# finmath/finmath-lib-cuda-extensions

Hardware: AMD Instinct MI355X
Metric: Monte-Carlo path-ops/sec (fused RandomVariable stream) (higher is better)
Workload: dtype f32

## Files before the change

### finmath-lib-cuda-extensions_amd/host/hip_backend.hpp

```cpp
#pragma once
#include <cstdlib>
#include <cstring>
#include <memory>
#include "lmm.hpp"

namespace fmhost {

class BrownianMotionFromMersenneRandomNumbersHip final : public BrownianMotion {
public:
    BrownianMotionFromMersenneRandomNumbersHip(TimeDiscretization td, int numberOfFactors, int64_t numberOfPaths, int seed, int64_t pathOffset = 0)
        : td_(std::move(td)), factors_(numberOfFactors), paths_(numberOfPaths), offset_(pathOffset), seed_(seed) {}
    RV getBrownianIncrement(int timeIndex, int factor) const override {
        std::call_once(generated_, [this] { generate(); });
        return inc_.at((size_t)timeIndex * factors_ + factor);
    }
    const TimeDiscretization& getTimeDiscretization() const override { return td_; }
    int getNumberOfFactors() const override { return factors_; }
    int64_t getNumberOfPaths() const override { return paths_; }
    int getSeed() const { return seed_; }
    RV getRandomVariableForConstant(double value) const override { return RandomVariableHip::of(-std::numeric_limits<double>::infinity(), value); }
private:
    void generate() const {
        const int steps = td_.getNumberOfTimeSteps();
        std::vector<double> dt((size_t)steps);
        for (int i = 0; i < steps; ++i) dt[(size_t)i] = td_.getTimeStep(i);
        std::vector<fmhip_vec> h((size_t)steps * factors_);
        check(fmhip_bm_generate_mersenne_device(seed_, steps, factors_, paths_, offset_, dt.data(), h.data()));
        inc_.reserve(h.size());
        for (int i = 0; i < steps; ++i)
            for (int f = 0; f < factors_; ++f)
                inc_.push_back(RandomVariableHip::of(td_.getTime(i + 1), DeviceVector(h[(size_t)i * factors_ + f]), paths_));
    }
    TimeDiscretization td_;
    int factors_;
    int64_t paths_, offset_;
    int seed_;
    mutable std::vector<RV> inc_;
    mutable std::once_flag generated_;
};

inline lmm::Backend makeHipBackend(const RandomVariableFactory* factory, const BrownianMotion* brownianMotion, int chunk = 0, int stepsPerLaunch = 0, int jacobianBatch = 0) {
    lmm::Backend be;
    be.factory = factory;
    be.brownianMotion = brownianMotion;
    if (!(std::getenv("FMHIP_LMM_FLUSH") && std::getenv("FMHIP_LMM_FLUSH")[0] == '0'))
        be.flush = [] { check(fmhip_flush()); };
    if (!(std::getenv("FMHIP_LMM_HOLD") && std::getenv("FMHIP_LMM_HOLD")[0] == '0'))
        be.hold = [](bool h) { check(fmhip_fusion_hold(h ? 1 : 0, nullptr)); };
    if (chunk > 0) be.chunk = chunk;
    if (stepsPerLaunch > 0) be.stepsPerLaunch = stepsPerLaunch;
    be.jacobianBatch = jacobianBatch > 0 ? jacobianBatch : 8;
    if (!(std::getenv("FMHIP_LMM_CLONE") && std::getenv("FMHIP_LMM_CLONE")[0] == '0')) {
        auto handleOf = [](const RV& x) {
            auto p = dynamic_cast<const RandomVariableHip*>(x.get());
            if (!p || p->isDeterministic()) throw std::runtime_error("graph replication over a value that is not a device vector");
            return p->deviceVector().handle();
        };
        be.clone = [handleOf](const std::vector<RV>& roots, const std::vector<RV>& leafFrom, const std::vector<std::vector<RV>>& leafTo,
                              const std::vector<std::vector<double>>* scalars) {
            const int nRoots = (int)roots.size(), nMap = (int)leafFrom.size(), nCopies = (int)leafTo.size();
            std::vector<fmhip_vec> r, lf, lt, out((size_t)nRoots * nCopies);
            for (const RV& x : roots) r.push_back(handleOf(x));
            for (const RV& x : leafFrom) lf.push_back(handleOf(x));
            for (const auto& row : leafTo) { if ((int)row.size() != nMap) throw std::runtime_error("graph replication: ragged operand map"); for (const RV& x : row) lt.push_back(handleOf(x)); }
            std::vector<double> sc;
            int nScalars = 0;
            if (scalars) { nScalars = (int)(*scalars)[0].size(); for (const auto& row : *scalars) { if ((int)row.size() != nScalars) throw std::runtime_error("graph replication: ragged scalar lists"); sc.insert(sc.end(), row.begin(), row.end()); } }
            check(fmhip_graph_clone(r.data(), nRoots, nCopies, lf.data(), lt.data(), nMap, scalars ? sc.data() : nullptr, nScalars, out.data()));
            std::vector<std::vector<RV>> copies((size_t)nCopies);
            for (int c = 0; c < nCopies; ++c)
                for (int k = 0; k < nRoots; ++k)
                    copies[(size_t)c].push_back(RandomVariableHip::of(roots[(size_t)k]->getFiltrationTime(), DeviceVector(out[(size_t)c * nRoots + k]), roots[(size_t)k]->size()));
            return copies;
        };
        be.recordedScalars = [handleOf](const std::vector<RV>& roots) {
            std::vector<fmhip_vec> r;
            for (const RV& x : roots) r.push_back(handleOf(x));
            int n = 0;
            check(fmhip_graph_scalars(r.data(), (int)r.size(), nullptr, 0, &n));
            std::vector<double> sc((size_t)n);
            check(fmhip_graph_scalars(r.data(), (int)r.size(), sc.data(), n, &n));
            return sc;
        };
    }
    if (!(std::getenv("FMHIP_LMM_DISCARD") && std::getenv("FMHIP_LMM_DISCARD")[0] == '0'))
        be.valuesNotNeeded = [](const std::vector<RV>& v) {
            std::vector<fmhip_vec> h;
            for (const RV& x : v) { auto p = dynamic_cast<const RandomVariableHip*>(x.get()); if (p && !p->isDeterministic()) h.push_back(p->deviceVector().handle()); }
            if (!h.empty()) check(fmhip_vec_give_up_values(h.data(), (int)h.size()));
        };
    be.launches = [] { fmhip_engine_stats_t s; check(fmhip_engine_stats(&s)); return (long long)s.kernel_launches; };
    be.averages = [](const std::vector<RV>& v) { return getAverages(v); };
    if (!(std::getenv("FMHIP_LMM_ASYNC") && std::getenv("FMHIP_LMM_ASYNC")[0] == '0'))
        be.expectationsRunPending = true;
    if (!(std::getenv("FMHIP_LMM_ASYNC") && std::getenv("FMHIP_LMM_ASYNC")[0] == '0'))
        be.averagesAsync = [](const std::vector<RV>& v) -> std::function<std::vector<double>()> {
            std::vector<fmhip_vec> h;
            int64_t n = 0;
            for (const RV& x : v) {
                auto p = dynamic_cast<const RandomVariableHip*>(x.get());
                if (!p || p->isDeterministic()) { const std::vector<double> now = getAverages(v); return [now] { return now; }; }
                h.push_back(p->deviceVector().handle()); n = p->size();
            }
            const int count = (int)h.size();
            fmhip_ticket ticket = 0;
            check(fmhip_reduce_moments_batch_begin(h.data(), count, nullptr, &ticket));
            struct Owner { fmhip_ticket t = 0; int count = 0; bool ended = false;
                           Owner() = default; Owner(const Owner&) = delete; Owner& operator=(const Owner&) = delete;
                           ~Owner() { if (!ended && t) { std::vector<fmhip_moments> drop((size_t)count); (void)fmhip_reduce_moments_batch_end(t, drop.data(), count); } } };
            auto owner = std::make_shared<Owner>();
            owner->t = ticket; owner->count = count;
            return [owner, count, n] {
                std::vector<fmhip_moments> m((size_t)count);
                owner->ended = true;
                check(fmhip_reduce_moments_batch_end(owner->t, m.data(), count));
                std::vector<double> out((size_t)count);
                for (int k = 0; k < count; ++k) out[(size_t)k] = m[(size_t)k].sum / (double)n;
                return out;
            };
        };
    return be;
}

}
```

### finmath-lib-cuda-extensions_amd/host/lmm.hpp

```cpp
#pragma once
#include <algorithm>
#include <chrono>
#include <cmath>
#include <cstdio>
#include <atomic>
#include <thread>
#include <cstdlib>
#include <functional>
#include <string>
#include <vector>

#include "random_variable.hpp"

namespace fmhost { namespace lmm {


inline const std::vector<double>& atmNormalVolatilities() {
    static const std::vector<double> v = {
        0.00151, 0.00169, 0.0021, 0.00248, 0.00291, 0.00329, 0.00365, 0.004, 0.00437, 0.00466, 0.00527, 0.00571,
        0.00604, 0.00625, 0.0016, 0.00174, 0.00217, 0.00264, 0.00314, 0.00355, 0.00398, 0.00433, 0.00469,
        0.00493, 0.00569, 0.00607, 0.00627, 0.00645, 0.00182, 0.00204, 0.00238, 0.00286, 0.00339, 0.00384,
        0.00424, 0.00456, 0.00488, 0.0052, 0.0059, 0.00623, 0.0064, 0.00654, 0.00205, 0.00235, 0.00272, 0.0032,
        0.00368, 0.00406, 0.00447, 0.00484, 0.00515, 0.00544, 0.00602, 0.00629, 0.0064, 0.00646, 0.00279,
        0.00319, 0.0036, 0.00396, 0.00436, 0.00469, 0.00503, 0.0053, 0.00557, 0.00582, 0.00616, 0.00628,
// ... 23 lines not shown
        const double w = (time - t[k - 1]) / (t[k] - t[k - 1]);
        return std::exp(logdf[k - 1] + w * (logdf[k] - logdf[k - 1]));
    }
    double forward(double fixing, double period) const { return (df(fixing) / df(fixing + period) - 1.0) / period; }
    static DiscountCurve bootstrap() {
        const double maturities[] = { 0.5, 1, 2, 3, 4, 5, 6, 7, 8, 9, 10, 11, 12, 15, 20, 25, 30, 35, 40, 45, 50 };
        const double rates[] = { -0.00216, -0.00208, -0.00222, -0.00216, -0.0019, -0.0014, -0.00072, 0.00011, 0.00103, 0.00196, 0.00285,
                                 0.00367, 0.0044, 0.00604, 0.00733, 0.00767, 0.00773, 0.00765, 0.00752, 0.007138, 0.007 };
        DiscountCurve c;
        for (int i = 0; i < 21; ++i) {
            const double M = maturities[i], r = rates[i];
            c.t.push_back(M); c.logdf.push_back(c.logdf.back());
            auto swapValue = [&](double ld) {
                c.logdf.back() = ld;
                double annuity = 0.0;
                if (M < 1.0) annuity = M * c.df(M);
                else for (double tp = 1.0; tp <= M + 1e-9; tp += 1.0) annuity += c.df(tp);
                return 1.0 - c.df(M) - r * annuity;
            };
            double lo = -3.0, hi = 1.0;
            for (int it = 0; it < 200; ++it) { const double mid = 0.5 * (lo + hi); if (swapValue(mid) > 0) lo = mid; else hi = mid; }
            c.logdf.back() = 0.5 * (lo + hi);
        }
        return c;
    }
};

struct Swaption {
    double exercise = 0; int numberOfPeriods = 0; double swapPeriodLength = 0.5;
    std::vector<double> swapTenor; double swaprate = 0, targetVolatility = 0, annuity = 0;
};

struct Market {
    DiscountCurve curve = DiscountCurve::bootstrap();
    double lastTime = 40.0, dt = 0.5;
    TimeDiscretization timeDiscretization{ 0.0, 80, 0.5 };
    std::vector<Swaption> swaptions;
    Market() {
        const auto& vols = atmNormalVolatilities();
        for (size_t e = 0; e < atmExpiryYears().size(); ++e)
            for (size_t k = 0; k < atmTenorYears().size(); ++k) {
                const double exercise = std::round(atmExpiryYears()[e] / 0.25) * 0.25, tenor = atmTenorYears()[k];
                if (exercise < 1.0) continue;
                if (exercise + tenor > lastTime + 1e-9) continue;
                Swaption s;
                s.exercise = exercise; s.numberOfPeriods = (int)std::lround(tenor / 0.5);
                for (int p = 0; p <= s.numberOfPeriods; ++p) s.swapTenor.push_back(exercise + p * 0.5);
                double floating = 0.0, annuity = 0.0;
                for (int p = 0; p < s.numberOfPeriods; ++p) {
                    const double d = curve.df(s.swapTenor[p + 1]);
                    floating += curve.forward(s.swapTenor[p], 0.5) * 0.5 * d; annuity += 0.5 * d;
                }
                s.swaprate = floating / annuity; s.annuity = annuity;
                s.targetVolatility = vols[e * atmTenorYears().size() + k];
                swaptions.push_back(std::move(s));
            }
    }
    int numberOfLibors() const { return timeDiscretization.getNumberOfTimeSteps(); }
};

struct VolatilityModel {
    std::vector<double> grid{ 0.0, 1.0, 2.0, 5.0, 10.0, 20.0, 30.0, 40.0 };
    std::vector<double> parameter = std::vector<double>(64, 0.50 / 100);
    int bin(double x) const { int k = 0; while (k < 7 && grid[(size_t)k] < x - 1e-12) ++k; return k; }
    int parameterIndex(double time, double maturity) const { return bin(time) * 8 + bin(maturity - time); }
    double volatility(double time, double maturity) const { return maturity <= time + 1e-12 ? 0.0 : parameter[(size_t)parameterIndex(time, maturity)]; }
    std::vector<int> activeParameters(const Market& m) const {
        std::vector<char> used(64, 0);
        const auto& td = m.timeDiscretization;
        for (int i = 0; i < td.getNumberOfTimeSteps(); ++i)
            for (int j = i + 1; j < m.numberOfLibors(); ++j) used[(size_t)parameterIndex(td.getTime(i), td.getTime(j))] = 1;
        std::vector<int> idx;
        for (int k = 0; k < 64; ++k) if (used[(size_t)k]) idx.push_back(k);
        return idx;
    }
};


struct Simulation {
    std::vector<std::vector<RV>> libor;
    std::vector<RV> numeraire;
};

struct Backend {
    const RandomVariableFactory* factory = nullptr;
    const BrownianMotion* brownianMotion = nullptr;
    std::function<void()> flush = [] {};
    std::function<void(bool)> hold = [](bool) {};
    std::function<long long()> launches = [] { return 0LL; };
    std::function<std::vector<double>(const std::vector<RV>&)> averages = [](const std::vector<RV>& v) {
        std::vector<double> a; for (const RV& x : v) a.push_back(x->getAverage()); return a; };
    std::function<std::function<std::vector<double>()>(const std::vector<RV>&)> averagesAsync;
    bool expectationsRunPending = false;
    std::function<void(const std::vector<RV>&)> valuesNotNeeded;
    int chunk = 7;
    int stepsPerLaunch = 4;
    std::function<std::vector<std::vector<RV>>(const std::vector<RV>& roots, const std::vector<RV>& leafFrom, const std::vector<std::vector<RV>>& leafTo,
                                               const std::vector<std::vector<double>>* scalars)> clone;
    std::function<std::vector<double>(const std::vector<RV>& roots)> recordedScalars;
    int jacobianBatch = 1;
    bool keepAllStates = false;
    int threads = 1;
};

inline std::vector<Simulation> simulateMany(const Market& m, const std::vector<const VolatilityModel*>& vols, const Backend& be, int lastTimeIndex,
                                            const std::vector<char>* keep = nullptr) {
    const auto& td = m.timeDiscretization;
    const int n = m.numberOfLibors();
    const double delta = m.dt;
    const size_t K = vols.size();
    std::vector<Simulation> sims(K);
    for (Simulation& sim : sims) {
        sim.libor.resize((size_t)lastTimeIndex + 1);
        sim.numeraire.resize((size_t)lastTimeIndex + 1);
        sim.libor[0].resize((size_t)n);
        for (int j = 0; j < n; ++j) sim.libor[0][(size_t)j] = be.factory->createRandomVariable(0.0, m.curve.forward(td.getTime(j), delta));
        sim.numeraire[0] = be.factory->createRandomVariable(0.0, 1.0);
    }
    std::vector<RV> factorSum(K);
    const int S = std::max(1, be.stepsPerLaunch);
    static int cloneChecks = 0;
    for (int i0 = 0; i0 < lastTimeIndex;) {
        int i1 = std::min(i0 + S, lastTimeIndex);
        static const bool endAtKept = std::getenv("FMHIP_LMM_GROUPS_END_AT_KEPT") && std::getenv("FMHIP_LMM_GROUPS_END_AT_KEPT")[0] == '1';
        if (keep && endAtKept) for (int s2 = i0 + 1; s2 < i1; ++s2) if ((*keep)[(size_t)s2]) { i1 = s2; break; }
        const bool cloning = K > 1 && S > 1 && keep && be.clone && i0 >= 2;
        const size_t Krec = cloning ? 1 : K;
        if (S > 1) be.hold(true);
        for (int i = i0; i < i1; ++i) {
            const double t = td.getTime(i), dt = td.getTimeStep(i);
            const RV dW = be.brownianMotion->getBrownianIncrement(i, 0);
            for (size_t k = 0; k < Krec; ++k) {
                auto& cur = sims[k].libor[(size_t)i];
                auto& nxt = sims[k].libor[(size_t)i + 1];
                nxt.resize((size_t)n);
                for (int j = 0; j <= i && j < n; ++j) nxt[(size_t)j] = cur[(size_t)j];
                factorSum[k] = nullptr;
            }
            for (int j0 = i + 1; j0 < n; j0 += be.chunk) {
                const int j1 = std::min(n, j0 + be.chunk);
                for (size_t k = 0; k < Krec; ++k) {
                    auto& cur = sims[k].libor[(size_t)i];
                    auto& nxt = sims[k].libor[(size_t)i + 1];
                    for (int j = j0; j < j1; ++j) {
                        const double lambda = vols[k]->volatility(t, td.getTime(j));
                        const RV& L = cur[(size_t)j];
                        const RV transform = be.factory->createRandomVariable(lambda * delta)->discount(L, delta);
                        factorSum[k] = factorSum[k] ? factorSum[k]->add(transform) : transform;
                        const RV drift = factorSum[k]->mult(lambda);
                        nxt[(size_t)j] = L->addProduct(drift, dt)->addProduct(dW, lambda);
                    }
                }
                if (S == 1 && j1 - j0 == be.chunk) be.flush();
            }
            for (size_t k = 0; k < Krec; ++k)
                sims[k].numeraire[(size_t)i + 1] = sims[k].numeraire[(size_t)i]->accrue(sims[k].libor[(size_t)i][(size_t)i], delta);
            for (size_t k = 0; k < Krec; ++k) factorSum[k] = nullptr;
        }
        if (cloning) {
            std::vector<RV> roots, leafFrom;
            for (int j = i0 + 1; j < n; ++j) roots.push_back(sims[0].libor[(size_t)i1][(size_t)j]);
            for (int i = i0; i < i1; ++i) roots.push_back(sims[0].numeraire[(size_t)i + 1]);
            for (int s2 = i0 + 1; s2 < i1; ++s2)
                if (!keep || (*keep)[(size_t)s2]) for (int j = s2; j < n; ++j) roots.push_back(sims[0].libor[(size_t)s2][(size_t)j]);
            for (int j = i0; j < n; ++j) leafFrom.push_back(sims[0].libor[(size_t)i0][(size_t)j]);
            leafFrom.push_back(sims[0].numeraire[(size_t)i0]);
            auto scalarsOf = [&](const VolatilityModel& vol) {
                std::vector<double> sc;
                for (int i = i0; i < i1; ++i) {
                    const double t = td.getTime(i), dt = td.getTimeStep(i);
                    for (int j = i + 1; j < n; ++j) {
                        const double lambda = vol.volatility(t, td.getTime(j));
                        sc.push_back(delta); sc.push_back(1.0); sc.push_back(lambda * delta); sc.push_back(lambda); sc.push_back(dt); sc.push_back(lambda);
                    }
                    sc.push_back(delta);
                }
                return sc;
            };
            if (cloneChecks < 64 && be.recordedScalars) {
                ++cloneChecks;
                if (be.recordedScalars(roots) != scalarsOf(*vols[0])) throw std::runtime_error("lmm: the scalar list of the replicated Euler steps does not match the recording");
            }
            std::vector<std::vector<RV>> leafTo(K - 1);
            std::vector<std::vector<double>> scalars(K - 1);
            for (size_t k = 1; k < K; ++k) {
                for (int j = i0; j < n; ++j) leafTo[k - 1].push_back(sims[k].libor[(size_t)i0][(size_t)j]);
                leafTo[k - 1].push_back(sims[k].numeraire[(size_t)i0]);
                scalars[k - 1] = scalarsOf(*vols[k]);
            }
            const std::vector<std::vector<RV>> copies = be.clone(roots, leafFrom, leafTo, &scalars);
            for (size_t k = 1; k < K; ++k) {
                auto& nxt = sims[k].libor[(size_t)i1];
                nxt.resize((size_t)n);
                for (int j = 0; j <= i0 && j < n; ++j) nxt[(size_t)j] = sims[k].libor[(size_t)i0][(size_t)j];
                size_t r = 0;
                for (int j = i0 + 1; j < n; ++j) nxt[(size_t)j] = copies[k - 1][r++];
                for (int i = i0; i < i1; ++i) sims[k].numeraire[(size_t)i + 1] = copies[k - 1][r++];
                for (int s2 = i0 + 1; s2 < i1; ++s2)
                    if (!keep || (*keep)[(size_t)s2]) { auto& mid = sims[k].libor[(size_t)s2]; mid.resize((size_t)n); for (int j = s2; j < n; ++j) mid[(size_t)j] = copies[k - 1][r++]; }
            }
        }
        if (keep)
            for (int i = i0; i < i1; ++i)
                if (!(*keep)[(size_t)i])
                    for (size_t k = 0; k < K; ++k) { sims[k].libor[(size_t)i].clear(); sims[k].libor[(size_t)i].shrink_to_fit(); }
        if (S > 1) be.hold(false);
        be.flush();
        i0 = i1;
    }
    return sims;
}

inline Simulation simulate(const Market& m, const VolatilityModel& vol, const Backend& be, int lastTimeIndex) {
    return std::move(simulateMany(m, { &vol }, be, lastTimeIndex)[0]);
}

inline RV swaptionValue(const Market& m, const Simulation& sim, const Swaption& s) {
    const auto& td = m.timeDiscretization;
    const int exerciseIndex = td.getTimeIndex(s.exercise);
    RV value;
    for (int p = s.numberOfPeriods - 1; p >= 0; --p) {
        const int j = td.getTimeIndex(s.swapTenor[(size_t)p]);
        const RV& libor = sim.libor[(size_t)exerciseIndex][(size_t)j];
        const RV payoff = libor->sub(s.swaprate)->mult(s.swapPeriodLength);
        value = (value ? value->add(payoff) : payoff)->discount(libor, s.swapPeriodLength);
    }
    return value->floor(0.0)->div(sim.numeraire[(size_t)exerciseIndex]);
}
inline double bachelierAtmImpliedVolatility(double optionValue, double optionMaturity, double annuity) {
    return optionValue * std::sqrt(2.0 * 3.14159265358979323846) / (annuity * std::sqrt(optionMaturity));
}

struct Valuation { std::vector<double> modelVolatility; double seconds_simulation = 0, seconds_valuation = 0; long long launches_simulation = 0, launches_valuation = 0; };

struct PendingValuations {
    std::vector<std::function<std::vector<double>()>> expectations;
    std::vector<Valuation> out;
};

inline std::vector<Valuation> evaluateManyFinish(const Market& m, PendingValuations& p) {
    for (size_t k = 0; k < p.out.size(); ++k) {
        const std::vector<double> optionValues = p.expectations[k]();
        for (size_t q = 0; q < m.swaptions.size(); ++q)
            p.out[k].modelVolatility.push_back(bachelierAtmImpliedVolatility(optionValues[q], m.swaptions[q].exercise, m.swaptions[q].annuity));
    }
    return std::move(p.out);
}

inline PendingValuations evaluateManyBegin(const Market& m, const std::vector<const VolatilityModel*>& vols, const Backend& be) {
    using clk = std::chrono::steady_clock;
    const size_t K = vols.size();
    PendingValuations pending;
    std::vector<Valuation>& out = pending.out;
    out.resize(K);
    int lastIndex = 0;
    for (const Swaption& s : m.swaptions) lastIndex = std::max(lastIndex, m.timeDiscretization.getTimeIndex(s.exercise));
    const auto t0 = clk::now();
    const long long l0 = be.launches();
    std::vector<char> keep((size_t)lastIndex + 1, 0);
    for (const Swaption& s : m.swaptions) keep[(size_t)m.timeDiscretization.getTimeIndex(s.exercise)] = 1;
    const std::vector<Simulation> sims = simulateMany(m, vols, be, lastIndex, be.keepAllStates ? nullptr : &keep);
    const auto t1 = clk::now();
    const long long l1 = be.launches();
    std::vector<std::vector<RV>> values(K);
    if (K > 1 && be.clone) {
        be.hold(true);
        values[0].reserve(m.swaptions.size());
        for (const Swaption& s : m.swaptions) values[0].push_back(swaptionValue(m, sims[0], s));
        std::vector<RV> leafFrom;
        std::vector<std::vector<RV>> leafTo(K - 1);
        for (int e = 0; e <= lastIndex; ++e) {
            if (!keep[(size_t)e]) continue;
            for (size_t k = 0; k < K; ++k) {
                std::vector<RV>& dst = k == 0 ? leafFrom : leafTo[k - 1];
                for (int j = e; j < m.numberOfLibors(); ++j) dst.push_back(sims[k].libor[(size_t)e][(size_t)j]);
                dst.push_back(sims[k].numeraire[(size_t)e]);
            }
        }
        const std::vector<std::vector<RV>> copies = be.clone(values[0], leafFrom, leafTo, nullptr);
        for (size_t k = 1; k < K; ++k) values[k] = copies[k - 1];
        be.hold(false);
        if (!(be.averagesAsync && be.expectationsRunPending)) be.flush();
    } else
    for (size_t k = 0; k < K; ++k) {
        be.hold(true);
        values[k].reserve(m.swaptions.size());
        for (const Swaption& s : m.swaptions) values[k].push_back(swaptionValue(m, sims[k], s));
        be.hold(false);
        if (!(be.averagesAsync && be.expectationsRunPending)) be.flush();
    }
    if (be.valuesNotNeeded) for (size_t k = 0; k < K; ++k) be.valuesNotNeeded(values[k]);
    for (size_t k = 0; k < K; ++k) {
        if (be.averagesAsync) pending.expectations.push_back(be.averagesAsync(values[k]));
        else { const std::vector<double> now = be.averages(values[k]); pending.expectations.push_back([now] { return now; }); }
    }
    const auto t2 = clk::now();
    for (size_t k = 0; k < K; ++k) {
        out[k].launches_simulation = (l1 - l0) / (long long)K; out[k].launches_valuation = (be.launches() - l1) / (long long)K;
        out[k].seconds_simulation = std::chrono::duration<double>(t1 - t0).count() / (double)K;
        out[k].seconds_valuation = std::chrono::duration<double>(t2 - t1).count() / (double)K;
    }
    return pending;
}

inline std::vector<Valuation> evaluateMany(const Market& m, const std::vector<const VolatilityModel*>& vols, const Backend& be) {
    PendingValuations p = evaluateManyBegin(m, vols, be);
    return evaluateManyFinish(m, p);
}

inline Valuation evaluate(const Market& m, const VolatilityModel& vol, const Backend& be) {
    return std::move(evaluateMany(m, { &vol }, be)[0]);
}


struct CalibrationResult {
    VolatilityModel model; int iterations = 0, evaluations = 0;
    double meanDeviation = 0, rmsDeviation = 0, initialRms = 0, seconds = 0, seconds_simulation = 0, seconds_valuation = 0;
    std::vector<double> modelVolatility;
};

inline bool solveSymmetric(std::vector<double> A, std::vector<double> b, int n, std::vector<double>& x) {
    for (int c = 0; c < n; ++c) {
        int piv = c;
        for (int r = c + 1; r < n; ++r) if (std::fabs(A[(size_t)r * n + c]) > std::fabs(A[(size_t)piv * n + c])) piv = r;
        if (std::fabs(A[(size_t)piv * n + c]) < 1e-300) return false;
        if (piv != c) { for (int k = 0; k < n; ++k) std::swap(A[(size_t)c * n + k], A[(size_t)piv * n + k]); std::swap(b[(size_t)c], b[(size_t)piv]); }
        for (int r = c + 1; r < n; ++r) {
            const double f = A[(size_t)r * n + c] / A[(size_t)c * n + c];
            for (int k = c; k < n; ++k) A[(size_t)r * n + k] -= f * A[(size_t)c * n + k];
            b[(size_t)r] -= f * b[(size_t)c];
        }
    }
    x.assign((size_t)n, 0.0);
    for (int r = n - 1; r >= 0; --r) { double s = b[(size_t)r]; for (int k = r + 1; k < n; ++k) s -= A[(size_t)r * n + k] * x[(size_t)k]; x[(size_t)r] = s / A[(size_t)r * n + r]; }
    return true;
}

inline CalibrationResult calibrate(const Market& m, const Backend& be, int maxIterations = 200, double accuracy = 1e-7,
                                   double lambda = 0.1, double parameterStep = 1e-4, bool verbose = false) {
    using clk = std::chrono::steady_clock;
    const auto start = clk::now();
    CalibrationResult res;
    VolatilityModel vol;
    const std::vector<int> active = vol.activeParameters(m);
    const int np = (int)active.size(), nr = (int)m.swaptions.size();
    auto residuals = [&](const VolatilityModel& v, std::vector<double>& r, std::vector<double>* modelVols) {
        const Valuation val = evaluate(m, v, be);
        res.evaluations++; res.seconds_simulation += val.seconds_simulation; res.seconds_valuation += val.seconds_valuation;
        r.resize((size_t)nr);
        for (int k = 0; k < nr; ++k) r[(size_t)k] = val.modelVolatility[(size_t)k] - m.swaptions[(size_t)k].targetVolatility;
        if (modelVols) *modelVols = val.modelVolatility;
    };
    auto sumsq = [](const std::vector<double>& r) { double s = 0; for (double x : r) s += x * x; return s; };
    std::vector<double> r, rTrial, modelVols;
    residuals(vol, r, &modelVols);
    double err = sumsq(r);
    res.initialRms = std::sqrt(err / nr);
    for (int it = 0; it < maxIterations; ++it) {
        std::vector<double> J((size_t)nr * np);
        struct InFlight { int a0 = 0, a1 = 0; std::vector<VolatilityModel> bumped; PendingValuations pending; bool valid = false; };
        auto collect = [&](InFlight& f) {
            if (!f.valid) return;
            const std::vector<Valuation> vals = evaluateManyFinish(m, f.pending);
            for (int a = f.a0; a < f.a1; ++a) {
                const Valuation& val = vals[(size_t)(a - f.a0)];
                res.evaluations++; res.seconds_simulation += val.seconds_simulation; res.seconds_valuation += val.seconds_valuation;
                for (int k = 0; k < nr; ++k) J[(size_t)k * np + a] = (val.modelVolatility[(size_t)k] - m.swaptions[(size_t)k].targetVolatility - r[(size_t)k]) / parameterStep;
            }
            f.valid = false;
        };
        if (be.threads > 1 && be.jacobianBatch <= 1) {
            const auto tj0 = clk::now();
            std::vector<Valuation> column((size_t)np);
            std::vector<std::string> failures((size_t)be.threads);
            std::atomic<int> next{ 0 };
            std::vector<std::thread> pool;
            for (int t = 0; t < be.threads; ++t)
                pool.emplace_back([&, t] {
                    try {
                        for (int a = next.fetch_add(1); a < np; a = next.fetch_add(1)) {
                            VolatilityModel bumped = vol;
                            bumped.parameter[(size_t)active[(size_t)a]] += parameterStep;
                            column[(size_t)a] = evaluate(m, bumped, be);
                        }
                    } catch (const std::exception& e) { failures[(size_t)t] = e.what(); }
                });
            for (std::thread& th : pool) th.join();
            if (std::getenv("FMHIP_LMM_TIMELINE")) std::fprintf(stderr, "[lmm timeline] iteration %d: %d columns on %d threads, %.3f … %.3f ms\n", it, np, be.threads, std::chrono::duration<double, std::milli>(tj0 - start).count(), std::chrono::duration<double, std::milli>(clk::now() - start).count());
            for (const std::string& f : failures) if (!f.empty()) throw std::runtime_error("a Jacobian column failed: " + f);
            for (int a = 0; a < np; ++a) {
                const Valuation& val = column[(size_t)a];
                res.evaluations++; res.seconds_simulation += val.seconds_simulation; res.seconds_valuation += val.seconds_valuation;
                for (int k = 0; k < nr; ++k) J[(size_t)k * np + a] = (val.modelVolatility[(size_t)k] - m.swaptions[(size_t)k].targetVolatility - r[(size_t)k]) / parameterStep;
            }
        } else {
        InFlight previous;
        for (int a0 = 0; a0 < np; a0 += std::max(1, be.jacobianBatch)) {
            const int a1 = std::min(np, a0 + std::max(1, be.jacobianBatch));
            InFlight current;
            current.a0 = a0; current.a1 = a1;
            current.bumped.assign((size_t)(a1 - a0), vol);
            std::vector<const VolatilityModel*> ptrs;
            for (int a = a0; a < a1; ++a) { current.bumped[(size_t)(a - a0)].parameter[(size_t)active[(size_t)a]] += parameterStep; ptrs.push_back(&current.bumped[(size_t)(a - a0)]); }
            static const bool timeline = std::getenv("FMHIP_LMM_TIMELINE") != nullptr;
            const auto tb0 = clk::now();
            try { current.pending = evaluateManyBegin(m, ptrs, be); current.valid = true; }
            catch (const std::exception& e) {
                if (ptrs.size() == 1 || std::string(e.what()).find("allocation") == std::string::npos) throw;
                if (verbose) std::fprintf(stderr, "  batch of %zu bumps does not fit (%s): evaluating them one at a time\n", ptrs.size(), e.what());
                be.flush();
                collect(previous);
                for (int a = a0; a < a1; ++a) {
                    const Valuation val = evaluate(m, current.bumped[(size_t)(a - a0)], be);
                    res.evaluations++; res.seconds_simulation += val.seconds_simulation; res.seconds_valuation += val.seconds_valuation;
                    for (int k = 0; k < nr; ++k) J[(size_t)k * np + a] = (val.modelVolatility[(size_t)k] - m.swaptions[(size_t)k].targetVolatility - r[(size_t)k]) / parameterStep;
                }
                continue;
            }
            const auto tb1 = clk::now();
            collect(previous);
            if (timeline) std::fprintf(stderr, "[lmm timeline] iteration %d batch from %d: begin %.3f … %.3f ms, previous collected at %.3f ms\n", it, a0,
                                       std::chrono::duration<double, std::milli>(tb0 - start).count(), std::chrono::duration<double, std::milli>(tb1 - start).count(),
                                       std::chrono::duration<double, std::milli>(clk::now() - start).count());
            previous = std::move(current);
        }
        collect(previous);
        }
        std::vector<double> JtJ((size_t)np * np, 0.0), Jtr((size_t)np, 0.0);
        for (int a = 0; a < np; ++a) {
            for (int b = 0; b < np; ++b) { double s = 0; for (int k = 0; k < nr; ++k) s += J[(size_t)k * np + a] * J[(size_t)k * np + b]; JtJ[(size_t)a * np + b] = s; }
            double s = 0; for (int k = 0; k < nr; ++k) s += J[(size_t)k * np + a] * r[(size_t)k]; Jtr[(size_t)a] = -s;
        }
        bool improved = false;
        for (int attempt = 0; attempt < 8 && !improved; ++attempt) {
            std::vector<double> A = JtJ, step;
            for (int a = 0; a < np; ++a) A[(size_t)a * np + a] += lambda * std::max(JtJ[(size_t)a * np + a], 1e-12);
            if (!solveSymmetric(A, Jtr, np, step)) { lambda *= 4; continue; }
            VolatilityModel v = vol;
            for (int a = 0; a < np; ++a) v.parameter[(size_t)active[(size_t)a]] += step[(size_t)a];
            std::vector<double> mv;
            const auto tt0 = clk::now();
            residuals(v, rTrial, &mv);
            static const bool timeline2 = std::getenv("FMHIP_LMM_TIMELINE") != nullptr;
            if (timeline2) std::fprintf(stderr, "[lmm timeline] iteration %d trial %d: %.3f … %.3f ms\n", it, attempt, std::chrono::duration<double, std::milli>(tt0 - start).count(),
                                        std::chrono::duration<double, std::milli>(clk::now() - start).count());
            const double e = sumsq(rTrial);
            if (e < err) { improved = true; const double rel = (err - e) / err; vol = v; r = rTrial; err = e; modelVols = mv; lambda = std::max(lambda / 3.0, 1e-9); if (rel < accuracy) it = maxIterations; }
            else lambda *= 4.0;
        }
        res.iterations++;
        if (verbose) std::fprintf(stderr, "  LM iteration %d: rms %.6e  lambda %.3g  evaluations %d\n", res.iterations, std::sqrt(err / nr), lambda, res.evaluations);
        if (!improved || std::sqrt(err / nr) < accuracy) break;
    }
    res.model = vol; res.modelVolatility = modelVols;
    double sum = 0; for (double x : r) sum += x;
    res.meanDeviation = sum / nr; res.rmsDeviation = std::sqrt(err / nr);
    res.seconds = std::chrono::duration<double>(clk::now() - start).count();
    return res;
}

}}
```

### finmath-lib-cuda-extensions_amd/host/lmm_hip_main.cpp

```cpp
#include <fstream>
#include <thread>
#include <csignal>
#include <execinfo.h>
#include <unistd.h>
#include <rccl/rccl.h>
#include "lmm_main_common.hpp"
#include "hip_backend.hpp"
using namespace fmhost;

static void ncclCheck(ncclResult_t r, const char* what) {
    if (r != ncclSuccess) throw std::runtime_error(std::string(what) + ": " + ncclGetErrorString(r));
}

static void fatalSignal(int sig) {
    void* frames[64];
    const int n = backtrace(frames, 64);
    const char msg[] = "lmm_hip: fatal signal, call stack:\n";
    (void)!write(2, msg, sizeof msg - 1);
    backtrace_symbols_fd(frames, n, 2);
    signal(sig, SIG_DFL);
    raise(sig);
}

int main(int argc, char** argv) {
    if (std::getenv("FMHIP_BACKTRACE")) { signal(SIGABRT, fatalSignal); signal(SIGSEGV, fatalSignal); signal(SIGBUS, fatalSignal); }
    const lmm::Options o = lmm::parseOptions(argc, argv);
    try {
        if (!o.devices.empty()) check(fmhip_init_devices(o.devices.data(), (int)o.devices.size()));
        else check(fmhip_init(-1));
        check(fmhip_set_fusion(1, nullptr));
        RandomVariableHipFactory factory;
        lmm::Market m;
        const int64_t pathOffset = o.pathOffset + (int64_t)o.rank * o.paths;
        BrownianMotionHip philox(m.timeDiscretization, 1, o.paths, o.seed, pathOffset);
        BrownianMotionFromMersenneRandomNumbers mersenne(m.timeDiscretization, 1, o.paths, (int)o.seed, &factory);
        if (o.brownian == "mersenne" && o.world > 1) throw std::runtime_error("--brownian mersenne is a sequential stream: not available with --world > 1 (mersenne-device is)");
        BrownianMotionFromMersenneRandomNumbersHip mersenneDevice(m.timeDiscretization, 1, o.paths, (int)o.seed, pathOffset);
        lmm::Backend be = makeHipBackend(&factory, (o.brownian == "mersenne") ? static_cast<const BrownianMotion*>(&mersenne)
                                                 : (o.brownian == "mersenne-device") ? static_cast<const BrownianMotion*>(&mersenneDevice) : &philox,
                                         o.chunk, o.stepsPerLaunch, o.jacobianBatch);

        if (o.finmathLike) {
            be.flush = [] {}; be.hold = [](bool) {}; be.clone = nullptr; be.recordedScalars = nullptr; be.averagesAsync = nullptr; be.expectationsRunPending = false;
            be.averages = [](const std::vector<RV>& v) { std::vector<double> a; for (const RV& x : v) a.push_back(x->getAverage()); return a; };
            be.jacobianBatch = 1; be.stepsPerLaunch = 1; be.chunk = 1 << 30; be.keepAllStates = true;
            if (o.threads > 1) {
                if (!o.devices.empty() || o.world > 1) throw std::runtime_error("--threads: one device, one process");
                check(fmhip_set_thread_engines(1, nullptr));
                be.threads = o.threads;
            }
        } else if (o.threads > 1) throw std::runtime_error("--threads belongs to --finmath-like (the native driver batches its Jacobian columns instead)");
        if (o.releaseLagMs > 0.0 || o.releaseLagBytes > 0) ReleaseLag::instance().start(o.releaseLagMs, (size_t)o.releaseLagBytes);
        ncclComm_t comm = nullptr;
        std::vector<std::pair<double*, hipEvent_t>> sparePinned;
        fmhip_vec sums = 0;
        long long collectives = 0;
        double collective_seconds = 0.0;
        if (o.world > 1 || !o.ncclIdFile.empty()) {
            if (o.ncclIdFile.empty()) throw std::runtime_error("--world needs --nccl-id-file");
            struct IdFile { uint64_t magic, nonce; ncclUniqueId id; } rec{};
            const uint64_t MAGIC = 0x464d4e43434c4944ull;
            if (o.rank == 0) {
                std::remove(o.ncclIdFile.c_str());
                rec.magic = MAGIC; rec.nonce = (uint64_t)o.ncclNonce;
                ncclCheck(ncclGetUniqueId(&rec.id), "ncclGetUniqueId");
                { std::ofstream f(o.ncclIdFile + ".tmp", std::ios::binary); f.write((const char*)&rec, sizeof rec); }
                std::rename((o.ncclIdFile + ".tmp").c_str(), o.ncclIdFile.c_str());
            } else {
                for (int tries = 0; ; ++tries) {
                    std::ifstream f(o.ncclIdFile, std::ios::binary);
                    if (f && f.read((char*)&rec, sizeof rec) && f.gcount() == (std::streamsize)sizeof rec && rec.magic == MAGIC && rec.nonce == (uint64_t)o.ncclNonce) break;
                    if (tries > 6000) throw std::runtime_error("timed out waiting for " + o.ncclIdFile);
                    std::this_thread::sleep_for(std::chrono::milliseconds(10));
                }
            }
            const ncclUniqueId id = rec.id;
            ncclCheck(ncclCommInitRank(&comm, o.world, id, o.rank), "ncclCommInitRank");
            if (o.rank == 0) std::remove(o.ncclIdFile.c_str());
            const int count = (int)m.swaptions.size();
            check(fmhip_vec_create_uninitialized((int64_t)count * 8 * o.world, &sums));
            void* stream = nullptr; check(fmhip_get_stream(&stream));
            const int64_t totalPaths = (int64_t)o.world * o.paths;
            const int world = o.world, rank = o.rank;
            struct Flight {
                fmhip_vec dev = 0; double* host = nullptr; hipEvent_t ev = nullptr;
                std::vector<std::pair<double*, hipEvent_t>>* spare = nullptr;
                ~Flight() { if (dev) fmhip_vec_release(dev); if (host && ev && spare) spare->push_back({ host, ev }); }
            };
            std::vector<std::pair<double*, hipEvent_t>>* const spare = &sparePinned;
            { const char* e = std::getenv("FMHIP_LMM_SHARDED_FROM_LAUNCHES"); be.expectationsRunPending = !(e && e[0] == '0'); }
            be.averagesAsync = [=, &collectives, &collective_seconds](const std::vector<RV>& v) -> std::function<std::vector<double>()> {
                std::vector<fmhip_vec> h;
                for (const RV& x : v) {
                    auto p = dynamic_cast<const RandomVariableHip*>(x.get());
                    if (!p || p->isDeterministic()) throw std::runtime_error("sharded expectation of a non-device value");
                    h.push_back(p->deviceVector().handle());
                }
                if ((int)h.size() != count) throw std::runtime_error("sharded expectation: unexpected product count");
                auto f = std::make_shared<Flight>();
                const size_t doubles = (size_t)count * 4 * (size_t)world;
                check(fmhip_vec_create_uninitialized((int64_t)doubles * 2, &f->dev));
                f->spare = spare;
                if (!spare->empty()) { f->host = spare->back().first; f->ev = spare->back().second; spare->pop_back(); }
                else if (hipHostMalloc((void**)&f->host, doubles * 8, hipHostMallocDefault) != hipSuccess || hipEventCreateWithFlags(&f->ev, hipEventDisableTiming) != hipSuccess)
                    throw std::runtime_error("pinned memory / event for a sharded expectation");
                void* dev = nullptr; check(fmhip_vec_device_ptr(f->dev, &dev));
                double* all = (double*)dev;
                check(fmhip_reduce_moments_batch_device(h.data(), count, nullptr, all + (size_t)rank * count * 4));
                ncclCheck(ncclAllGather(all + (size_t)rank * count * 4, all, (size_t)count * 4, ncclDouble, comm, (hipStream_t)stream), "ncclAllGather");
                if (hipMemcpyAsync(f->host, all, doubles * 8, hipMemcpyDeviceToHost, (hipStream_t)stream) != hipSuccess || hipEventRecord(f->ev, (hipStream_t)stream) != hipSuccess)
                    throw std::runtime_error("enqueueing the read-back of a sharded expectation");
                ++collectives;
                return [f, count, world, totalPaths, &collective_seconds] {
                    const auto t0 = std::chrono::steady_clock::now();
                    if (hipEventSynchronize(f->ev) != hipSuccess) throw std::runtime_error("waiting for a sharded expectation");
                    collective_seconds += std::chrono::duration<double>(std::chrono::steady_clock::now() - t0).count();
                    std::vector<double> out((size_t)count);
                    for (int k = 0; k < count; ++k) {
                        double total = 0.0;
                        for (int r = 0; r < world; ++r) total += f->host[((size_t)r * count + k) * 4];
                        out[(size_t)k] = total / (double)totalPaths;
                    }
                    return out;
                };
            };
            be.averages = [=, &collectives, &collective_seconds](const std::vector<RV>& v) {
                std::vector<fmhip_vec> h;
                for (const RV& x : v) {
                    auto p = dynamic_cast<const RandomVariableHip*>(x.get());
                    if (!p || p->isDeterministic()) throw std::runtime_error("sharded expectation of a non-device value");
                    h.push_back(p->deviceVector().handle());
                }
                if ((int)h.size() != count) throw std::runtime_error("sharded expectation: unexpected product count");
                void* dev = nullptr; check(fmhip_vec_device_ptr(sums, &dev));
                double* all = (double*)dev;
                check(fmhip_reduce_moments_batch_device(h.data(), count, nullptr, all + (size_t)rank * count * 4));
                const auto t0 = std::chrono::steady_clock::now();
                ncclCheck(ncclAllGather(all + (size_t)rank * count * 4, all, (size_t)count * 4, ncclDouble, comm, (hipStream_t)stream), "ncclAllGather");
                ++collectives;
                std::vector<float> raw((size_t)count * 8 * world);
                check(fmhip_vec_read_float(sums, raw.data(), (int64_t)raw.size()));
                collective_seconds += std::chrono::duration<double>(std::chrono::steady_clock::now() - t0).count();
// ... 70 lines not shown
```

### finmath-lib-cuda-extensions_amd/host/lmm_main_common.hpp

```cpp
#pragma once
#include <vector>
#include <cstdlib>
#include <cstring>
#include <string>
#include "lmm.hpp"

namespace fmhost { namespace lmm {

struct Options {
    int64_t paths = 10000; int64_t seed = 31415; int maxIterations = 200; std::string mode = "calibrate"; bool verbose = false;
    int64_t pathOffset = 0; int evaluations = 1;
    int warmupEvaluations = 0;
    int world = 1, rank = 0; std::string ncclIdFile; long long ncclNonce = 0;
    std::vector<int> devices;
    int chunk = 0;
    int stepsPerLaunch = 0;
    int jacobianBatch = 0;
    std::string brownian = "philox";
    int threads = 1;
    double releaseLagMs = 0.0;
    long long releaseLagBytes = 0;
    bool finmathLike = false;
    bool profile = false;
};
inline Options parseOptions(int argc, char** argv) {
    Options o;
    for (int i = 1; i < argc; ++i) {
        const std::string a = argv[i];
        auto next = [&]() -> const char* { if (i + 1 >= argc) { std::fprintf(stderr, "missing value for %s\n", a.c_str()); std::exit(2); } return argv[++i]; };
        if (a == "--paths") o.paths = std::atoll(next());
        else if (a == "--seed") o.seed = std::atoll(next());
        else if (a == "--max-iterations") o.maxIterations = std::atoi(next());
        else if (a == "--mode") o.mode = next();
        else if (a == "--evaluations") o.evaluations = std::atoi(next());
        else if (a == "--warmup-evaluations") o.warmupEvaluations = std::atoi(next());
        else if (a == "--path-offset") o.pathOffset = std::atoll(next());
        else if (a == "--world") o.world = std::atoi(next());
        else if (a == "--devices") { std::string list = next(); size_t p0 = 0; while (p0 <= list.size()) { const size_t q = list.find(',', p0); o.devices.push_back(std::atoi(list.substr(p0, q == std::string::npos ? std::string::npos : q - p0).c_str())); if (q == std::string::npos) break; p0 = q + 1; } }
        else if (a == "--rank") o.rank = std::atoi(next());
        else if (a == "--nccl-id-file") o.ncclIdFile = next();
        else if (a == "--nccl-nonce") o.ncclNonce = std::atoll(next());
        else if (a == "--profile") o.profile = true;
        else if (a == "--finmath-like") o.finmathLike = true;
        else if (a == "--threads") o.threads = std::atoi(next());
        else if (a == "--release-lag") o.releaseLagMs = std::atof(next());
        else if (a == "--release-lag-bytes") o.releaseLagBytes = std::atoll(next());
        else if (a == "--brownian") o.brownian = next();
        else if (a == "--jacobian-batch") o.jacobianBatch = std::atoi(next());
        else if (a == "--chunk") o.chunk = std::atoi(next());
        else if (a == "--steps-per-launch") o.stepsPerLaunch = std::atoi(next());
        else if (a == "--verbose") o.verbose = true;
        else { std::fprintf(stderr, "unknown option %s\n", a.c_str()); std::exit(2); }
    }
    return o;
}

inline void runAndReport(const Options& o, const Backend& be, const char* backendName, const std::function<std::string()>& extraJson) {
    Market m;
    if (o.mode == "evaluate") {
        VolatilityModel vol;
        Valuation v;
        double sim = 0, val = 0;
        const int K = std::max(1, o.jacobianBatch);
        for (int k = 0; k < o.evaluations; k += K) {
            const int kk = std::min(K, o.evaluations - k);
            const std::vector<Valuation> vs = evaluateMany(m, std::vector<const VolatilityModel*>((size_t)kk, &vol), be);
            for (const Valuation& x : vs) { sim += x.seconds_simulation; val += x.seconds_valuation; }
            v = vs.back();
        }
        std::printf("{\"backend\": \"%s\", \"mode\": \"evaluate\", \"paths\": %lld, \"swaptions\": %zu, \"evaluations\": %d, "
                    "\"seconds_simulation_per_evaluation\": %.6f, \"seconds_valuation_per_evaluation\": %.6f, \"launches_simulation\": %lld, \"launches_valuation\": %lld%s, \"model_volatility\": [",
                    backendName, (long long)o.paths, m.swaptions.size(), o.evaluations, sim / o.evaluations, val / o.evaluations, v.launches_simulation, v.launches_valuation, extraJson().c_str());
        for (size_t k = 0; k < v.modelVolatility.size(); ++k) std::printf("%s%.17g", k ? ", " : "", v.modelVolatility[k]);
        std::printf("]}\n");
        return;
    }
    const CalibrationResult r = calibrate(m, be, o.maxIterations, 1e-7, 0.1, 1e-4, o.verbose);
    std::printf("{\"backend\": \"%s\", \"mode\": \"calibrate\", \"paths\": %lld, \"swaptions\": %zu, \"active_parameters\": %zu, "
                "\"iterations\": %d, \"evaluations\": %d, \"seconds\": %.4f, \"seconds_simulation\": %.4f, \"seconds_valuation\": %.4f, "
                "\"initial_rms\": %.6e, \"rms_deviation\": %.6e, \"mean_deviation\": %.6e%s, \"parameters\": [",
                backendName, (long long)o.paths, m.swaptions.size(), VolatilityModel().activeParameters(m).size(), r.iterations, r.evaluations,
                r.seconds, r.seconds_simulation, r.seconds_valuation, r.initialRms, r.rmsDeviation, r.meanDeviation, extraJson().c_str());
    for (size_t k = 0; k < r.model.parameter.size(); ++k) std::printf("%s%.17g", k ? ", " : "", r.model.parameter[k]);
    std::printf("]}\n");
}

}}
```

Measured before the change: 4269 billion.

## Reuse base-point simulation states for Jacobian bumps in LMM calibration

In calibration, each bumped-parameter simulation now starts from the base point's kept state at the group containing the parameter's first use, instead of from time zero. Swaptions whose exercise precedes that point reuse the base model volatilities and are not revalued. Jacobian batches are regrouped by a small dynamic program that weighs simulated groups against batch size. This spends memory on keeping group-start states and adds bookkeeping, and it is disabled for multi-device runs.

```diff
diff --git a/finmath-lib-cuda-extensions_amd/host/hip_backend.hpp b/finmath-lib-cuda-extensions_amd/host/hip_backend.hpp
--- a/finmath-lib-cuda-extensions_amd/host/hip_backend.hpp
+++ b/finmath-lib-cuda-extensions_amd/host/hip_backend.hpp
@@ -50,6 +50,7 @@
     if (chunk > 0) be.chunk = chunk;
     if (stepsPerLaunch > 0) be.stepsPerLaunch = stepsPerLaunch;
     be.jacobianBatch = jacobianBatch > 0 ? jacobianBatch : 8;
+    be.basePoint = lmm::basePointFromEnvironment(true);
     if (!(std::getenv("FMHIP_LMM_CLONE") && std::getenv("FMHIP_LMM_CLONE")[0] == '0')) {
         auto handleOf = [](const RV& x) {
             auto p = dynamic_cast<const RandomVariableHip*>(x.get());
diff --git a/finmath-lib-cuda-extensions_amd/host/lmm.hpp b/finmath-lib-cuda-extensions_amd/host/lmm.hpp
--- a/finmath-lib-cuda-extensions_amd/host/lmm.hpp
+++ b/finmath-lib-cuda-extensions_amd/host/lmm.hpp
@@ -129,6 +129,11 @@
     std::vector<RV> numeraire;
 };
 
+inline bool basePointFromEnvironment(bool otherwise) {
+    const char* e = std::getenv("FMHIP_LMM_BASE_POINT");
+    return e && e[0] ? e[0] != '0' : otherwise;
+}
+
 struct Backend {
     const RandomVariableFactory* factory = nullptr;
     const BrownianMotion* brownianMotion = nullptr;
@@ -147,19 +152,40 @@
     std::function<std::vector<double>(const std::vector<RV>& roots)> recordedScalars;
     int jacobianBatch = 1;
     bool keepAllStates = false;
+    bool basePoint = basePointFromEnvironment(false);
     int threads = 1;
 };
 
+inline int groupEnd(const Backend& be, int i0, int lastTimeIndex, const std::vector<char>* keep) {
+    int i1 = std::min(i0 + std::max(1, be.stepsPerLaunch), lastTimeIndex);
+    static const bool endAtKept = std::getenv("FMHIP_LMM_GROUPS_END_AT_KEPT") && std::getenv("FMHIP_LMM_GROUPS_END_AT_KEPT")[0] == '1';
+    if (keep && endAtKept) for (int s2 = i0 + 1; s2 < i1; ++s2) if ((*keep)[(size_t)s2]) { i1 = s2; break; }
+    return i1;
+}
+inline int groupStart(const Backend& be, int i, int lastTimeIndex, const std::vector<char>* keep) {
+    for (int i0 = 0; i0 < lastTimeIndex;) {
+        const int i1 = groupEnd(be, i0, lastTimeIndex, keep);
+        if (i < i1) return i0;
+        i0 = i1;
+    }
+    return lastTimeIndex;
+}
+
 inline std::vector<Simulation> simulateMany(const Market& m, const std::vector<const VolatilityModel*>& vols, const Backend& be, int lastTimeIndex,
-                                            const std::vector<char>* keep = nullptr) {
+                                            const std::vector<char>* keep = nullptr, const Simulation* base = nullptr, int start = 0, bool keepGroupStarts = false) {
     const auto& td = m.timeDiscretization;
     const int n = m.numberOfLibors();
     const double delta = m.dt;
     const size_t K = vols.size();
     std::vector<Simulation> sims(K);
+    if (!base) start = 0;
+    if (start < 0 || start > lastTimeIndex) throw std::runtime_error("lmm: a simulation cannot start at this time index");
+    if (start > 0 && (base->libor.size() <= (size_t)start || base->libor[(size_t)start].size() != (size_t)n || !base->numeraire[(size_t)start]))
+        throw std::runtime_error("lmm: the base simulation has not kept the state the columns start from");
     for (Simulation& sim : sims) {
         sim.libor.resize((size_t)lastTimeIndex + 1);
         sim.numeraire.resize((size_t)lastTimeIndex + 1);
+        if (start > 0) { sim.libor[(size_t)start] = base->libor[(size_t)start]; sim.numeraire[(size_t)start] = base->numeraire[(size_t)start]; continue; }
         sim.libor[0].resize((size_t)n);
         for (int j = 0; j < n; ++j) sim.libor[0][(size_t)j] = be.factory->createRandomVariable(0.0, m.curve.forward(td.getTime(j), delta));
         sim.numeraire[0] = be.factory->createRandomVariable(0.0, 1.0);
@@ -167,10 +193,8 @@
     std::vector<RV> factorSum(K);
     const int S = std::max(1, be.stepsPerLaunch);
     static int cloneChecks = 0;
-    for (int i0 = 0; i0 < lastTimeIndex;) {
-        int i1 = std::min(i0 + S, lastTimeIndex);
-        static const bool endAtKept = std::getenv("FMHIP_LMM_GROUPS_END_AT_KEPT") && std::getenv("FMHIP_LMM_GROUPS_END_AT_KEPT")[0] == '1';
-        if (keep && endAtKept) for (int s2 = i0 + 1; s2 < i1; ++s2) if ((*keep)[(size_t)s2]) { i1 = s2; break; }
+    for (int i0 = start; i0 < lastTimeIndex;) {
+        const int i1 = groupEnd(be, i0, lastTimeIndex, keep);
         const bool cloning = K > 1 && S > 1 && keep && be.clone && i0 >= 2;
         const size_t Krec = cloning ? 1 : K;
         if (S > 1) be.hold(true);
@@ -249,7 +273,7 @@
         }
         if (keep)
             for (int i = i0; i < i1; ++i)
-                if (!(*keep)[(size_t)i])
+                if (!(*keep)[(size_t)i] && !(keepGroupStarts && i == i0))
                     for (size_t k = 0; k < K; ++k) { sims[k].libor[(size_t)i].clear(); sims[k].libor[(size_t)i].shrink_to_fit(); }
         if (S > 1) be.hold(false);
         be.flush();
@@ -280,13 +304,42 @@
 
 struct Valuation { std::vector<double> modelVolatility; double seconds_simulation = 0, seconds_valuation = 0; long long launches_simulation = 0, launches_valuation = 0; };
 
+struct BasePoint {
+    Simulation simulation;
+    std::vector<double> modelVolatility;
+};
+
+struct ExerciseDates {
+    int lastIndex = 0;
+    std::vector<char> keep;
+    explicit ExerciseDates(const Market& m) {
+        for (const Swaption& s : m.swaptions) lastIndex = std::max(lastIndex, m.timeDiscretization.getTimeIndex(s.exercise));
+        keep.assign((size_t)lastIndex + 1, 0);
+        for (const Swaption& s : m.swaptions) keep[(size_t)m.timeDiscretization.getTimeIndex(s.exercise)] = 1;
+    }
+};
+
 struct PendingValuations {
     std::vector<std::function<std::vector<double>()>> expectations;
     std::vector<Valuation> out;
+    bool fromBasePoint = false;
+    std::vector<int> valued;
+    int start = 0;
+    std::vector<double> baseVolatility;
 };
 
 inline std::vector<Valuation> evaluateManyFinish(const Market& m, PendingValuations& p) {
     for (size_t k = 0; k < p.out.size(); ++k) {
+        if (p.fromBasePoint) {
+            p.out[k].modelVolatility = p.baseVolatility;
+            if (p.valued.empty()) continue;
+            const std::vector<double> optionValues = p.expectations[k]();
+            for (size_t r = 0; r < p.valued.size(); ++r) {
+                const size_t q = (size_t)p.valued[r];
+                p.out[k].modelVolatility[q] = bachelierAtmImpliedVolatility(optionValues[r], m.swaptions[q].exercise, m.swaptions[q].annuity);
+            }
+            continue;
+        }
         const std::vector<double> optionValues = p.expectations[k]();
         for (size_t q = 0; q < m.swaptions.size(); ++q)
             p.out[k].modelVolatility.push_back(bachelierAtmImpliedVolatility(optionValues[q], m.swaptions[q].exercise, m.swaptions[q].annuity));
@@ -294,30 +347,41 @@
     return std::move(p.out);
 }
 
-inline PendingValuations evaluateManyBegin(const Market& m, const std::vector<const VolatilityModel*>& vols, const Backend& be) {
+inline PendingValuations evaluateManyBegin(const Market& m, const std::vector<const VolatilityModel*>& vols, const Backend& be,
+                                           const BasePoint* base = nullptr, int firstUse = 0, BasePoint* produce = nullptr) {
     using clk = std::chrono::steady_clock;
     const size_t K = vols.size();
     PendingValuations pending;
     std::vector<Valuation>& out = pending.out;
     out.resize(K);
-    int lastIndex = 0;
-    for (const Swaption& s : m.swaptions) lastIndex = std::max(lastIndex, m.timeDiscretization.getTimeIndex(s.exercise));
+    const ExerciseDates dates(m);
+    const int lastIndex = dates.lastIndex;
+    const std::vector<char>& keep = dates.keep;
+    if (produce && (K != 1 || be.keepAllStates)) throw std::runtime_error("lmm: a base point is one parameter set's, with the states no product reads released");
+    std::vector<int> valued;
+    for (size_t q = 0; q < m.swaptions.size(); ++q)
+        if (!base || m.timeDiscretization.getTimeIndex(m.swaptions[q].exercise) > firstUse) valued.push_back((int)q);
+    int start = 0;
+    if (base) {
+        if (be.keepAllStates) throw std::runtime_error("lmm: no base point for a caller that keeps every state");
+        start = groupStart(be, firstUse, lastIndex, &keep);
+        pending.fromBasePoint = true; pending.valued = valued; pending.start = start; pending.baseVolatility = base->modelVolatility;
+        if (valued.empty()) return pending;
+    }
     const auto t0 = clk::now();
     const long long l0 = be.launches();
-    std::vector<char> keep((size_t)lastIndex + 1, 0);
-    for (const Swaption& s : m.swaptions) keep[(size_t)m.timeDiscretization.getTimeIndex(s.exercise)] = 1;
-    const std::vector<Simulation> sims = simulateMany(m, vols, be, lastIndex, be.keepAllStates ? nullptr : &keep);
+    std::vector<Simulation> sims = simulateMany(m, vols, be, lastIndex, be.keepAllStates ? nullptr : &keep, base ? &base->simulation : nullptr, start, produce != nullptr);
     const auto t1 = clk::now();
     const long long l1 = be.launches();
     std::vector<std::vector<RV>> values(K);
     if (K > 1 && be.clone) {
         be.hold(true);
-        values[0].reserve(m.swaptions.size());
-        for (const Swaption& s : m.swaptions) values[0].push_back(swaptionValue(m, sims[0], s));
+        values[0].reserve(valued.size());
+        for (const int q : valued) values[0].push_back(swaptionValue(m, sims[0], m.swaptions[(size_t)q]));
         std::vector<RV> leafFrom;
         std::vector<std::vector<RV>> leafTo(K - 1);
         for (int e = 0; e <= lastIndex; ++e) {
-            if (!keep[(size_t)e]) continue;
+            if (!keep[(size_t)e] || (base && e <= firstUse)) continue;
             for (size_t k = 0; k < K; ++k) {
                 std::vector<RV>& dst = k == 0 ? leafFrom : leafTo[k - 1];
                 for (int j = e; j < m.numberOfLibors(); ++j) dst.push_back(sims[k].libor[(size_t)e][(size_t)j]);
@@ -331,8 +395,8 @@
     } else
     for (size_t k = 0; k < K; ++k) {
         be.hold(true);
-        values[k].reserve(m.swaptions.size());
-        for (const Swaption& s : m.swaptions) values[k].push_back(swaptionValue(m, sims[k], s));
+        values[k].reserve(valued.size());
+        for (const int q : valued) values[k].push_back(swaptionValue(m, sims[k], m.swaptions[(size_t)q]));
         be.hold(false);
         if (!(be.averagesAsync && be.expectationsRunPending)) be.flush();
     }
@@ -347,6 +411,7 @@
         out[k].seconds_simulation = std::chrono::duration<double>(t1 - t0).count() / (double)K;
         out[k].seconds_valuation = std::chrono::duration<double>(t2 - t1).count() / (double)K;
     }
+    if (produce) produce->simulation = std::move(sims[0]);
     return pending;
 }
 
@@ -364,6 +429,7 @@
     VolatilityModel model; int iterations = 0, evaluations = 0;
     double meanDeviation = 0, rmsDeviation = 0, initialRms = 0, seconds = 0, seconds_simulation = 0, seconds_valuation = 0;
     std::vector<double> modelVolatility;
+    long long timeStepsNotSimulated = 0, productsNotValued = 0;
 };
 
 inline bool solveSymmetric(std::vector<double> A, std::vector<double> b, int n, std::vector<double>& x) {
@@ -391,8 +457,37 @@
     VolatilityModel vol;
     const std::vector<int> active = vol.activeParameters(m);
     const int np = (int)active.size(), nr = (int)m.swaptions.size();
-    auto residuals = [&](const VolatilityModel& v, std::vector<double>& r, std::vector<double>* modelVols) {
-        const Valuation val = evaluate(m, v, be);
+    const bool useBasePoint = be.basePoint && !be.keepAllStates && be.threads <= 1;
+    const ExerciseDates dates(m);
+    std::vector<int> firstUse((size_t)np, dates.lastIndex), startOf((size_t)np, 0);
+    if (useBasePoint)
+        for (int a = 0; a < np; ++a) {
+            const auto& td = m.timeDiscretization;
+            for (int i = 0; i < dates.lastIndex && firstUse[(size_t)a] == dates.lastIndex; ++i)
+                for (int j = i + 1; j < m.numberOfLibors(); ++j)
+                    if (vol.parameterIndex(td.getTime(i), td.getTime(j)) == active[(size_t)a]) { firstUse[(size_t)a] = i; break; }
+            startOf[(size_t)a] = groupStart(be, firstUse[(size_t)a], dates.lastIndex, &dates.keep);
+        }
+    std::vector<int> batchEnd((size_t)np, np);
+    if (useBasePoint) {
+        auto groupsFrom = [&](int i0) { int g = 0; while (i0 < dates.lastIndex) { i0 = groupEnd(be, i0, dates.lastIndex, &dates.keep); ++g; } return g; };
+        const int cap = std::max(1, be.jacobianBatch);
+        std::vector<long long> cost((size_t)np + 1, 0);
+        for (int a = np - 1; a >= 0; --a) {
+            cost[(size_t)a] = -1;
+            int first = startOf[(size_t)a];
+            for (int e = a + 1; e <= std::min(np, a + cap); ++e) {
+                first = std::min(first, startOf[(size_t)e - 1]);
+                const long long c = (long long)groupsFrom(first) * (e - a + 5) + cost[(size_t)e];
+                if (cost[(size_t)a] < 0 || c <= cost[(size_t)a]) { cost[(size_t)a] = c; batchEnd[(size_t)a] = e; }
+            }
+        }
+    }
+    BasePoint base;
+    auto residuals = [&](const VolatilityModel& v, std::vector<double>& r, std::vector<double>* modelVols, BasePoint* produce) {
+        PendingValuations p = evaluateManyBegin(m, { &v }, be, nullptr, 0, produce);
+        const Valuation val = std::move(evaluateManyFinish(m, p)[0]);
+        if (produce) produce->modelVolatility = val.modelVolatility;
         res.evaluations++; res.seconds_simulation += val.seconds_simulation; res.seconds_valuation += val.seconds_valuation;
         r.resize((size_t)nr);
         for (int k = 0; k < nr; ++k) r[(size_t)k] = val.modelVolatility[(size_t)k] - m.swaptions[(size_t)k].targetVolatility;
@@ -400,7 +495,7 @@
     };
     auto sumsq = [](const std::vector<double>& r) { double s = 0; for (double x : r) s += x * x; return s; };
     std::vector<double> r, rTrial, modelVols;
-    residuals(vol, r, &modelVols);
+    residuals(vol, r, &modelVols, useBasePoint ? &base : nullptr);
     double err = sumsq(r);
     res.initialRms = std::sqrt(err / nr);
     for (int it = 0; it < maxIterations; ++it) {
@@ -442,8 +537,10 @@
             }
         } else {
         InFlight previous;
-        for (int a0 = 0; a0 < np; a0 += std::max(1, be.jacobianBatch)) {
-            const int a1 = std::min(np, a0 + std::max(1, be.jacobianBatch));
+        for (int a0 = 0, a1 = 0; a0 < np; a0 = a1) {
+            a1 = useBasePoint ? batchEnd[(size_t)a0] : std::min(np, a0 + std::max(1, be.jacobianBatch));
+            int batchFirstUse = firstUse[(size_t)a0];
+            for (int a = a0 + 1; a < a1; ++a) batchFirstUse = std::min(batchFirstUse, firstUse[(size_t)a]);
             InFlight current;
             current.a0 = a0; current.a1 = a1;
             current.bumped.assign((size_t)(a1 - a0), vol);
@@ -451,7 +548,14 @@
             for (int a = a0; a < a1; ++a) { current.bumped[(size_t)(a - a0)].parameter[(size_t)active[(size_t)a]] += parameterStep; ptrs.push_back(&current.bumped[(size_t)(a - a0)]); }
             static const bool timeline = std::getenv("FMHIP_LMM_TIMELINE") != nullptr;
             const auto tb0 = clk::now();
-            try { current.pending = evaluateManyBegin(m, ptrs, be); current.valid = true; }
+            try {
+                current.pending = evaluateManyBegin(m, ptrs, be, useBasePoint ? &base : nullptr, batchFirstUse);
+                current.valid = true;
+                if (useBasePoint) {
+                    res.timeStepsNotSimulated += (long long)(a1 - a0) * current.pending.start;
+                    res.productsNotValued += (long long)(a1 - a0) * (nr - (long long)current.pending.valued.size());
+                }
+            }
             catch (const std::exception& e) {
                 if (ptrs.size() == 1 || std::string(e.what()).find("allocation") == std::string::npos) throw;
                 if (verbose) std::fprintf(stderr, "  batch of %zu bumps does not fit (%s): evaluating them one at a time\n", ptrs.size(), e.what());
@@ -466,9 +570,9 @@
             }
             const auto tb1 = clk::now();
             collect(previous);
-            if (timeline) std::fprintf(stderr, "[lmm timeline] iteration %d batch from %d: begin %.3f … %.3f ms, previous collected at %.3f ms\n", it, a0,
+            if (timeline) std::fprintf(stderr, "[lmm timeline] iteration %d batch from %d to %d: begin %.3f … %.3f ms, previous collected at %.3f ms, %lld launches so far\n", it, a0, a1,
                                        std::chrono::duration<double, std::milli>(tb0 - start).count(), std::chrono::duration<double, std::milli>(tb1 - start).count(),
-                                       std::chrono::duration<double, std::milli>(clk::now() - start).count());
+                                       std::chrono::duration<double, std::milli>(clk::now() - start).count(), be.launches());
             previous = std::move(current);
         }
         collect(previous);
@@ -486,13 +590,14 @@
             VolatilityModel v = vol;
             for (int a = 0; a < np; ++a) v.parameter[(size_t)active[(size_t)a]] += step[(size_t)a];
             std::vector<double> mv;
+            BasePoint trial;
             const auto tt0 = clk::now();
-            residuals(v, rTrial, &mv);
+            residuals(v, rTrial, &mv, useBasePoint ? &trial : nullptr);
             static const bool timeline2 = std::getenv("FMHIP_LMM_TIMELINE") != nullptr;
             if (timeline2) std::fprintf(stderr, "[lmm timeline] iteration %d trial %d: %.3f … %.3f ms\n", it, attempt, std::chrono::duration<double, std::milli>(tt0 - start).count(),
                                         std::chrono::duration<double, std::milli>(clk::now() - start).count());
             const double e = sumsq(rTrial);
-            if (e < err) { improved = true; const double rel = (err - e) / err; vol = v; r = rTrial; err = e; modelVols = mv; lambda = std::max(lambda / 3.0, 1e-9); if (rel < accuracy) it = maxIterations; }
+            if (e < err) { improved = true; const double rel = (err - e) / err; base = std::move(trial); vol = v; r = rTrial; err = e; modelVols = mv; lambda = std::max(lambda / 3.0, 1e-9); if (rel < accuracy) it = maxIterations; }
             else lambda *= 4.0;
         }
         res.iterations++;
diff --git a/finmath-lib-cuda-extensions_amd/host/lmm_hip_main.cpp b/finmath-lib-cuda-extensions_amd/host/lmm_hip_main.cpp
--- a/finmath-lib-cuda-extensions_amd/host/lmm_hip_main.cpp
+++ b/finmath-lib-cuda-extensions_amd/host/lmm_hip_main.cpp
@@ -58,6 +58,7 @@
         double collective_seconds = 0.0;
         if (o.world > 1 || !o.ncclIdFile.empty()) {
             if (o.ncclIdFile.empty()) throw std::runtime_error("--world needs --nccl-id-file");
+            be.basePoint = false;
             struct IdFile { uint64_t magic, nonce; ncclUniqueId id; } rec{};
             const uint64_t MAGIC = 0x464d4e43434c4944ull;
             if (o.rank == 0) {
diff --git a/finmath-lib-cuda-extensions_amd/host/lmm_main_common.hpp b/finmath-lib-cuda-extensions_amd/host/lmm_main_common.hpp
--- a/finmath-lib-cuda-extensions_amd/host/lmm_main_common.hpp
+++ b/finmath-lib-cuda-extensions_amd/host/lmm_main_common.hpp
@@ -78,9 +78,11 @@
     const CalibrationResult r = calibrate(m, be, o.maxIterations, 1e-7, 0.1, 1e-4, o.verbose);
     std::printf("{\"backend\": \"%s\", \"mode\": \"calibrate\", \"paths\": %lld, \"swaptions\": %zu, \"active_parameters\": %zu, "
                 "\"iterations\": %d, \"evaluations\": %d, \"seconds\": %.4f, \"seconds_simulation\": %.4f, \"seconds_valuation\": %.4f, "
-                "\"initial_rms\": %.6e, \"rms_deviation\": %.6e, \"mean_deviation\": %.6e%s, \"parameters\": [",
+                "\"initial_rms\": %.6e, \"rms_deviation\": %.6e, \"mean_deviation\": %.6e, "
+                "\"base_point\": {\"time_steps_not_simulated\": %lld, \"products_not_valued\": %lld}%s, \"parameters\": [",
                 backendName, (long long)o.paths, m.swaptions.size(), VolatilityModel().activeParameters(m).size(), r.iterations, r.evaluations,
-                r.seconds, r.seconds_simulation, r.seconds_valuation, r.initialRms, r.rmsDeviation, r.meanDeviation, extraJson().c_str());
+                r.seconds, r.seconds_simulation, r.seconds_valuation, r.initialRms, r.rmsDeviation, r.meanDeviation,
+                r.timeStepsNotSimulated, r.productsNotValued, extraJson().c_str());
     for (size_t k = 0; k < r.model.parameter.size(); ++k) std::printf("%s%.17g", k ? ", " : "", r.model.parameter[k]);
     std::printf("]}\n");
 }
```

After: 4189 billion. 1.9% lower.
